# ateme-developers/SVT-AV1-1

Measured on AMD Instinct MI355X. Metric: 64x64 SAD-search blocks/sec, higher is better.
Workload: dtype u8; 1 GPU; configs[1]: 64x64 full-pel SAD hierarchical ME (centre check + HME L0/L1/L2 + 64x64-area full-pel search of 85 square PUs), 1080p 8-bit, one reference list

## Files before the change

### svt-av1-1_amd/csrc/me_fullpel.hip

```cpp
#include <hip/hip_runtime.h>
#include <stdint.h>

#include "me_kernels.h"
#include "me_wave_reduce.h"

namespace svthip {

namespace {
#include "me_fullpel_impl.h"
}

__global__ void __launch_bounds__(256, SVTHIP_FULLPEL_MIN_WAVES) fullpel85_kernel(
    const uint8_t* __restrict__ src_plane, uint32_t src_stride, const uint8_t* __restrict__ ref_plane,
    uint32_t ref_stride, const int32_t* __restrict__ desc, uint32_t n_sb, uint32_t* __restrict__ out_sad,
    uint32_t* __restrict__ out_mv)
{
    extern __shared__ __attribute__((aligned(16))) uint8_t smem[];
    const uint32_t sb = xcd_item(blockIdx.x, n_sb);
    if (sb >= n_sb) return;
    if ((desc[6 * sb + 4] & 15) == 0) fullpel85_sb<true>(src_plane, src_stride, ref_plane, ref_stride, desc + 6 * sb, sb, out_sad, out_mv, smem);
    else fullpel85_sb<false>(src_plane, src_stride, ref_plane, ref_stride, desc + 6 * sb, sb, out_sad, out_mv, smem);
}

}
```

### svt-av1-1_amd/csrc/me_fullpel_impl.h

```cpp
#pragma once


constexpr int kPitch = SVTHIP_FULLPEL_LDS_PITCH;

__device__ __forceinline__ uint64_t pack64(uint32_t lo, uint32_t hi) { return ((uint64_t)hi << 32) | lo; }

struct __attribute__((packed, aligned(1))) unaligned_u32 { uint32_t v; };
struct __attribute__((packed, aligned(1))) unaligned_u32x4 { uint32_t v[4]; };

__device__ __forceinline__ uint32_t min3u(uint32_t a, uint32_t b, uint32_t c)
{
    uint32_t r;
    asm("v_min3_u32 %0, %1, %2, %3" : "=v"(r) : "v"(a), "v"(b), "v"(c));
    return r;
}

__device__ __forceinline__ uint32_t track4(uint32_t best, uint64_t acc, const uint32_t* idx, uint32_t himask)
{
    const uint32_t lo = (uint32_t)acc, hi = (uint32_t)(acc >> 32);
    uint32_t k0 = (lo << 16) | idx[0];
    uint32_t k1 = (lo & himask) | idx[1];
    uint32_t k2 = (hi << 16) | idx[2];
    uint32_t k3 = (hi & himask) | idx[3];
    best = min3u(best, k0, k1);
    best = min3u(best, k2, k3);
    return best;
}

__device__ __forceinline__ uint32_t pk_min_u16(uint32_t a, uint32_t b)
{
    uint32_t r;
    asm("v_pk_min_u16 %0, %1, %2" : "=v"(r) : "v"(a), "v"(b));
    return r;
}

__device__ __forceinline__ uint32_t wave_min_u32(uint32_t v)
{
#pragma unroll
    for (int m = 1; m < 64; m <<= 1) {
        uint32_t o = __shfl_xor(v, m);
        v = o < v ? o : v;
    }
    return v;
}

__device__ __forceinline__ unsigned long long wave_min_u64(unsigned long long v)
{
#pragma unroll
    for (int m = 1; m < 64; m <<= 1) {
        unsigned long long o = __shfl_xor(v, m);
        v = o < v ? o : v;
    }
    return v;
}

__device__ __forceinline__ uint32_t mv_word(int x, int y)
{
    return ((uint32_t)(uint16_t)(y * 4) << 16) | (uint32_t)(uint16_t)(x * 4);
}


template <bool CLS>
__device__ __forceinline__ void fullpel85_sb(const uint8_t* __restrict__ src_plane, uint32_t src_stride,
                                             const uint8_t* __restrict__ ref_plane, uint32_t ref_stride, const int32_t* d, uint32_t sbi,
                                             uint32_t* __restrict__ out_sad, uint32_t* __restrict__ out_mv, uint8_t* smem)
{
    uint32_t* xch = reinterpret_cast<uint32_t*>(smem);
    unsigned long long* best64_lds = reinterpret_cast<unsigned long long*>(smem + 16384);
    uint8_t* win = smem + 16384 + 64;

    const int tid = threadIdx.x;
    const int lane = tid & 63;
    const int Q = __builtin_amdgcn_readfirstlane(tid >> 6);
    const int Qx = Q & 1, Qy = Q >> 1;

    const int src_off = __builtin_amdgcn_readfirstlane(d[0]);
    const int ref_off = __builtin_amdgcn_readfirstlane(d[1]);
    const int xo = __builtin_amdgcn_readfirstlane(d[2]), yo = __builtin_amdgcn_readfirstlane(d[3]);
    const int sw = __builtin_amdgcn_readfirstlane(d[4]), sh = __builtin_amdgcn_readfirstlane(d[5]);
    const int n_xg = (sw + 15) >> 4;
    const uint32_t inv_xg = (65536u + (uint32_t)n_xg - 1u) / (uint32_t)n_xg;

#ifdef SVTHIP_FP_STAGE_PRIO
    __builtin_amdgcn_s_setprio(3);
#endif
    {
        const uint8_t* base = ref_plane + ref_off;
        const int rows = sh + 63;
        const int ndw_valid = (sw + 63 + 3) >> 2;
        constexpr int q_row = kPitch >> 4;
        const int total = rows * q_row;
        for (int i = tid; i < total; i += 256) {
            const int r = i / q_row;
            const int c4 = i - r * q_row;
            const uint8_t* p = base + (size_t)r * ref_stride + 16 * c4;
            const int left = ndw_valid - 4 * c4;
            uint32_t t[4] = {0u, 0u, 0u, 0u};
            if (left >= 4) {
                const unaligned_u32x4 u = *reinterpret_cast<const unaligned_u32x4*>(p);
                t[0] = u.v[0]; t[1] = u.v[1]; t[2] = u.v[2]; t[3] = u.v[3];
            } else if (left > 0) {
#pragma unroll
                for (int k = 0; k < 3; k++)
                    if (k < left) t[k] = reinterpret_cast<const unaligned_u32*>(p + 4 * k)->v;
            }
            reinterpret_cast<uint4*>(win)[i] = make_uint4(t[0], t[1], t[2], t[3]);
        }
        if (tid == 0) *best64_lds = ~0ull;
    }
    __syncthreads();
#ifdef SVTHIP_FP_STAGE_PRIO
    __builtin_amdgcn_s_setprio(0);
#endif

    const uint32_t* src4 = reinterpret_cast<const uint32_t*>(src_plane + src_off + (size_t)(32 * Qy) * src_stride + 32 * Qx);
    const int sstride4 = src_stride >> 2;

    uint32_t rsv[4][2] = {{0, 0}, {0, 0}, {0, 0}, {0, 0}};
    if constexpr (CLS) {
        const int p = lane >> 2, zz = p >> 2, k = p & 3, px = 16 * (zz & 1) + 8 * (k & 1), py = 16 * (zz >> 1) + 8 * (k >> 1);
        const uint32_t* sp = src4 + (size_t)py * sstride4 + (px >> 2);
#pragma unroll
        for (int r = 0; r < 4; r++) {
            rsv[r][0] = sp[(size_t)(2 * r) * sstride4];
            rsv[r][1] = sp[(size_t)(2 * r) * sstride4 + 1];
        }
    }

    uint32_t best8[16], best16[4], best32 = 0xffffffffu;
#pragma unroll
    for (int i = 0; i < 16; i++) best8[i] = 0xffffffffu;
#pragma unroll
    for (int i = 0; i < 4; i++) best16[i] = 0xffffffffu;
    uint32_t best64_raw = 0xffffffffu, best64_idx = 0;

    const uint32_t himask = 0xffff0000u;
    const int n_items = n_xg * sh;
    const int n_iter = (n_items + 63) >> 6;

    for (int it = 0; it < n_iter; it++) {
        int pg = it * 64 + lane;
        const bool lane_valid = pg < n_items;
        if (!lane_valid) pg = 0;
        const int y = (int)(((uint32_t)pg * inv_xg) >> 16);
        const int xg = pg - y * n_xg;

        uint32_t idx[16];
        const uint32_t idx0 = (uint32_t)(y * 128 + 16 * xg);
        if ((sw & 15) == 0) {
#pragma unroll
            for (int i = 0; i < 16; i++) idx[i] = idx0 + (uint32_t)i;
        } else {
#pragma unroll
            for (int i = 0; i < 16; i++) idx[i] = (16 * xg + i < sw) ? idx0 + (uint32_t)i : 0xffffffffu;
        }

        uint32_t s16lo[4][4], s16hi[4][4];

        const uint8_t* wbase = win + (y + 32 * Qy) * kPitch + 16 * xg + 32 * Qx;

        uint4 An, Bn;
        uint32_t Sn[4];
        {
            An = *reinterpret_cast<const uint4*>(wbase);
            Bn = *reinterpret_cast<const uint4*>(wbase + 16);
#pragma unroll
            for (int h = 0; h < 4; h++) Sn[h] = src4[h];
        }
#pragma unroll
        for (int zz = 0; zz < 4; zz++) {
            uint64_t acc[4][4];

#pragma unroll
            for (int r8 = 0; r8 < 8; r8++) {
                const uint4 A = An, B = Bn;
                const uint32_t W[8] = {A.x, A.y, A.z, A.w, B.x, B.y, B.z, B.w};
                const uint32_t S[4] = {Sn[0], Sn[1], Sn[2], Sn[3]};
                asm volatile("" ::"v"(A.x), "v"(A.y), "v"(A.z), "v"(A.w), "v"(B.x), "v"(B.y), "v"(B.z), "v"(B.w), "s"(S[0]), "s"(S[1]), "s"(S[2]), "s"(S[3]));
                __builtin_amdgcn_sched_barrier(0);
                {
                    const int nstep = zz * 8 + r8 + 1;
                    if (nstep < 32) {
                        const int nzz = nstep >> 3, nr8 = nstep & 7, nC = nzz & 1, nR = nzz >> 1;
                        const uint8_t* p = wbase + (16 * nR + 2 * nr8) * kPitch + 16 * nC;
                        An = *reinterpret_cast<const uint4*>(p);
                        Bn = *reinterpret_cast<const uint4*>(p + 16);
                        const uint32_t* srow = src4 + (16 * nR + 2 * nr8) * sstride4 + 4 * nC;
#pragma unroll
                        for (int h = 0; h < 4; h++) Sn[h] = srow[h];
                    }
                    __builtin_amdgcn_sched_barrier(0);
                }
                const int krow = (r8 >> 2) * 2;
#pragma unroll
                for (int q = 0; q < 4; q++)
#pragma unroll
                    for (int h = 0; h < 4; h++) {
                        const int k = krow + (h >> 1);
                        const bool first = ((r8 & 3) == 0) && ((h & 1) == 0);
                        acc[k][q] = __builtin_amdgcn_qsad_pk_u16_u8(pack64(W[q + h], W[q + h + 1]), S[h],
                                                                    first ? 0ull : acc[k][q]);
                    }
            }

#pragma unroll
            for (int k = 0; k < 4; k++) {
                if constexpr (CLS) {
                    const uint32_t mlo = pk_min_u16(pk_min_u16((uint32_t)acc[k][0], (uint32_t)acc[k][1]), pk_min_u16((uint32_t)acc[k][2], (uint32_t)acc[k][3]));
                    const uint32_t mhi = pk_min_u16(pk_min_u16((uint32_t)(acc[k][0] >> 32), (uint32_t)(acc[k][1] >> 32)),
                                                    pk_min_u16((uint32_t)(acc[k][2] >> 32), (uint32_t)(acc[k][3] >> 32)));
                    best8[4 * zz + k] = track4(best8[4 * zz + k], pack64(mlo, mhi), &idx[0], himask);
                } else {
#pragma unroll
                    for (int q = 0; q < 4; q++) best8[4 * zz + k] = track4(best8[4 * zz + k], acc[k][q], &idx[4 * q], himask);
                }
            }

#pragma unroll
            for (int q = 0; q < 4; q++) {
                const uint32_t lo = (uint32_t)acc[0][q] + (uint32_t)acc[1][q] + (uint32_t)acc[2][q] + (uint32_t)acc[3][q];
                const uint32_t hi = (uint32_t)(acc[0][q] >> 32) + (uint32_t)(acc[1][q] >> 32) +
                                    (uint32_t)(acc[2][q] >> 32) + (uint32_t)(acc[3][q] >> 32);
                best16[zz] = track4(best16[zz], pack64(lo, hi), &idx[4 * q], himask);
                s16lo[zz][q] = lo;
                s16hi[zz][q] = hi;
            }
        }

        uint32_t s32acc[16];
#pragma unroll
        for (int q = 0; q < 4; q++) {
            const uint32_t a_lo = s16lo[0][q] + s16lo[1][q], b_lo = s16lo[2][q] + s16lo[3][q];
            const uint32_t a_hi = s16hi[0][q] + s16hi[1][q], b_hi = s16hi[2][q] + s16hi[3][q];
            s32acc[4 * q + 0] = (a_lo & 0xffffu) + (b_lo & 0xffffu);
            s32acc[4 * q + 1] = (a_lo >> 16) + (b_lo >> 16);
            s32acc[4 * q + 2] = (a_hi & 0xffffu) + (b_hi & 0xffffu);
            s32acc[4 * q + 3] = (a_hi >> 16) + (b_hi >> 16);
        }

#pragma unroll
        for (int i = 0; i < 16; i += 2) {
            uint32_t k0 = (s32acc[i] << 14) | idx[i];
            uint32_t k1 = (s32acc[i + 1] << 14) | idx[i + 1];
            best32 = min3u(best32, k0, k1);
        }

        __syncthreads();
        {
            uint4* dst = reinterpret_cast<uint4*>(xch + Q * 1024 + lane * 4);
#pragma unroll
            for (int q = 0; q < 4; q++) dst[q * 64] = make_uint4(s32acc[4 * q], s32acc[4 * q + 1], s32acc[4 * q + 2], s32acc[4 * q + 3]);
        }
        __syncthreads();
        {
            uint4 s = make_uint4(0, 0, 0, 0);
#pragma unroll
            for (int w = 0; w < 4; w++) {
                const uint4 v = *reinterpret_cast<const uint4*>(xch + w * 1024 + Q * 256 + lane * 4);
                s.x += v.x; s.y += v.y; s.z += v.z; s.w += v.w;
            }
            const uint32_t sv[4] = {s.x, s.y, s.z, s.w};
            const int xbase = 16 * xg + 4 * Q;
            const uint32_t ibase = (uint32_t)(y * 128 + xbase);
#pragma unroll
            for (int j = 0; j < 4; j++) {
                const bool better = (sv[j] < best64_raw) && lane_valid && (xbase + j < sw);
                best64_raw = better ? sv[j] : best64_raw;
                best64_idx = better ? (ibase + j) : best64_idx;
            }
        }
    }

    uint32_t* osad = out_sad + (size_t)85 * sbi;
    uint32_t* omv = out_mv + (size_t)85 * sbi;

    const uint32_t g8 = wave_min_scatter<16>(best8, lane);
    const uint32_t top[8] = {best16[0], best16[1], best16[2], best16[3], best32, 0xffffffffu, 0xffffffffu, 0xffffffffu};
    const uint32_t g16 = wave_min_scatter<8, 5>(top, lane);
    const unsigned long long k64 = wave_min_u64(((unsigned long long)best64_raw << 32) | best64_idx);

    if constexpr (CLS) {
        const int p = lane >> 2, q = lane & 3;
        const uint32_t key = (uint32_t)__shfl((int)g8, p);
        const uint32_t s = key >> 16, id = key & 0xffffu;
        const int y = (int)(id >> 7), xb = (int)(id & 0x70u);
        const int zz = p >> 2, k = p & 3, px = 16 * (zz & 1) + 8 * (k & 1), py = 16 * (zz >> 1) + 8 * (k >> 1);
        const uint8_t* wp = win + (y + 32 * Qy + py) * kPitch + xb + 4 * q + 32 * Qx + px;
        uint64_t a = 0;
#pragma unroll
        for (int r = 0; r < 4; r++) {
            const uint32_t* w = reinterpret_cast<const uint32_t*>(wp + 2 * r * kPitch);
            const uint32_t w0 = w[0], w1 = w[1], w2 = w[2];
            a = __builtin_amdgcn_qsad_pk_u16_u8(pack64(w0, w1), rsv[r][0], a);
            a = __builtin_amdgcn_qsad_pk_u16_u8(pack64(w1, w2), rsv[r][1], a);
        }
        const uint32_t lo = (uint32_t)a, hi = (uint32_t)(a >> 32);
        uint32_t first = (lo & 0xffffu) == s ? 0u : (lo >> 16) == s ? 1u : (hi & 0xffffu) == s ? 2u : (hi >> 16) == s ? 3u : 64u;
        first += 4u * (uint32_t)q;
        first = min(first, (uint32_t)__shfl_xor((int)first, 1));
        first = min(first, (uint32_t)__shfl_xor((int)first, 2));
        if (q == 0) {
            const int pu = 21 + 16 * Q + p;
            osad[pu] = 2u * s;
            omv[pu] = mv_word(xo + xb + (int)first, yo + y);
        }
    }
    if (lane < 21 && !(CLS && lane < 16)) {
        const uint32_t key = lane < 16 ? g8 : g16;
        const int pu = lane < 16 ? 21 + 16 * Q + lane : lane < 20 ? 5 + 4 * Q + (lane - 16) : 1 + Q;
        const uint32_t raw = lane == 20 ? key >> 14 : key >> 16, id = key & 0x3fffu;
        osad[pu] = 2u * raw;
        omv[pu] = mv_word(xo + (int)(id & 127u), yo + (int)(id >> 7));
    }
    if (lane == 0) atomicMin(best64_lds, k64);
    __syncthreads();
    if (tid == 0) {
        const unsigned long long k = *best64_lds;
        const uint32_t raw = (uint32_t)(k >> 32), id = (uint32_t)k;
        osad[0] = 2u * raw;
        omv[0] = mv_word(xo + (int)(id & 127u), yo + (int)(id >> 7));
    }
}
```

### svt-av1-1_amd/csrc/svthip_abi.hip

```cpp
#include <hip/hip_runtime.h>
#include <stdint.h>
#include <stdio.h>
#include <stdlib.h>
#include <string.h>

#include <mutex>
#include <new>

#include "../../include/svtav1_hip.h"
#include "me_kernels.h"

namespace {

thread_local char g_err[512] = "";

int32_t fail(int32_t code, const char* fmt, const char* a = "", int b = 0)
{
    snprintf(g_err, sizeof(g_err), fmt, a, b);
    return code;
}

#define HIP_TRY(expr)                                                                              \
    do {                                                                                           \
        hipError_t e_ = (expr);                                                                    \
        if (e_ != hipSuccess) return fail(SVTHIP_ERR_DEVICE, "%s failed at line %d", hipGetErrorString(e_), __LINE__); \
    } while (0)

}

struct svthip_ctx {
    int device;
    hipStream_t stream;
    void* scratch[18];
    size_t scratch_bytes[18];
    hipStream_t inter_stream;
    hipStream_t scratch_stream;
    hipEvent_t scratch_event;
    int32_t opt[SVTHIP_OPT_COUNT];
    uint32_t sb_table_w, sb_table_h;
};

namespace {

std::once_flag g_attr_once[16];
hipError_t g_attr_status[16];

void set_kernel_attrs(int device)
{
    const void* kernels[] = {reinterpret_cast<const void*>(svthip::fullpel85_kernel),  reinterpret_cast<const void*>(svthip::fullpel209_kernel),
                             reinterpret_cast<const void*>(svthip::bipred_pack_kernel), reinterpret_cast<const void*>(svthip::bipred_nsq_pack_kernel),
                             reinterpret_cast<const void*>(svthip::subpel_planes_kernel), svthip::convolve_compound_kernel_ptr(0),
                             svthip::convolve_compound_kernel_ptr(1),                     svthip::convolve_compound_kernel_ptr(2),
                             svthip::convolve_compound_kernel_ptr(3),                     svthip::convolve_compound_count_kernel_ptr(0),
                             svthip::convolve_compound_count_kernel_ptr(1),               svthip::convolve_compound_count_kernel_ptr(2),
                             svthip::convolve_compound_count_kernel_ptr(3)};
    hipError_t st = hipSuccess;
    for (const void* k : kernels) {
        hipFuncAttributes fa;
        hipError_t e = hipFuncGetAttributes(&fa, k);
        if (e == hipSuccess) e = hipFuncSetAttribute(k, hipFuncAttributeMaxDynamicSharedMemorySize, 160 * 1024 - (int)fa.sharedSizeBytes);
        if (e != hipSuccess) st = e;
    }
    g_attr_status[device] = st;
}

int32_t enter(svthip_ctx* c)
{
    if (!c) return fail(SVTHIP_ERR_BAD_PARAMETER, "null context%s", "");
    HIP_TRY(hipSetDevice(c->device));
    return SVTHIP_OK;
}
#define ENTER(ctx)                         \
    do {                                   \
        int32_t rc_ = enter(ctx);          \
        if (rc_) return rc_;               \
    } while (0)

int32_t scratch_on_stream(svthip_ctx* c, hipStream_t s)
{
    if (c->scratch_stream && c->scratch_stream != s) {
        HIP_TRY(hipEventRecord(c->scratch_event, c->scratch_stream));
        HIP_TRY(hipStreamWaitEvent(s, c->scratch_event, 0));
    }
    c->scratch_stream = s;
    return SVTHIP_OK;
}

int32_t ensure_scratch(svthip_ctx* c, int slot, size_t bytes)
{
    if (c->scratch_bytes[slot] >= bytes) return SVTHIP_OK;
    hipStream_t os = c->scratch_stream ? c->scratch_stream : c->stream;
    if (c->scratch[slot] && hipFreeAsync(c->scratch[slot], os) != hipSuccess) {
        (void)hipGetLastError();
        HIP_TRY(hipFree(c->scratch[slot]));
    }
    c->scratch[slot] = nullptr;
    c->scratch_bytes[slot] = 0;
    size_t want = bytes + bytes / 4 + 4096;
    if (hipMallocAsync(&c->scratch[slot], want, os) != hipSuccess) {
        (void)hipGetLastError();
        c->scratch[slot] = nullptr;
        return fail(SVTHIP_ERR_INSUFFICIENT_RESOURCES, "hipMallocAsync of %s scratch failed (slot %d)", "device", slot);
    }
    c->scratch_bytes[slot] = want;
    c->scratch_stream = os;
    if (slot == 9) {
        c->sb_table_w = c->sb_table_h = 0;
        HIP_TRY(hipMemsetAsync(c->scratch[9], 0, want, os));
    }
    return SVTHIP_OK;
}

size_t me_chain_bytes(size_t n, uint32_t n_pu)
{
    const size_t desc_b = sizeof(svthip_fullpel_desc) * n, arr_b = sizeof(uint32_t) * n_pu * n;
    const size_t state_b = ((sizeof(int16_t) * SVTHIP_HME_STATE_INT16 * n) + 15) & ~(size_t)15;
    return 2 * desc_b + 4 * arr_b + state_b + 64;
}
size_t me_pred_bytes(size_t n, uint32_t n_pu) { return 2 * (size_t)(n_pu == 209 ? 14 : 4) * 4096 * n; }

struct HostPoolLayout {
    uint32_t fs, qs, ss;
    size_t fb, qb, sb, per;
};
HostPoolLayout host_pool_layout(uint32_t w, uint32_t h)
{
    auto al = [](size_t v) { return (v + 15) & ~(size_t)15; };
    HostPoolLayout L;
    L.fs = w + 136; L.qs = (w >> 1) + 64; L.ss = (w >> 2) + 32;
    L.fb = al((size_t)L.fs * (h + 136)); L.qb = al((size_t)L.qs * ((h >> 1) + 64)); L.sb = al((size_t)L.ss * ((h >> 2) + 32));
    L.per = L.fb + L.qb + L.sb;
    return L;
}

int32_t ensure_sb_table(svthip_ctx* c, uint32_t w, uint32_t h, hipStream_t s)
{
    const uint32_t nx = (w + 63) / 64, ny = (h + 63) / 64, n_sb = nx * ny;
    int32_t rc;
    if ((rc = ensure_scratch(c, 9, sizeof(svthip_sb_origin) * n_sb))) return rc;
    if (c->sb_table_w == w && c->sb_table_h == h) return SVTHIP_OK;
    svthip_sb_origin* sbs = new (std::nothrow) svthip_sb_origin[n_sb];
    if (!sbs) return fail(SVTHIP_ERR_INSUFFICIENT_RESOURCES, "out of host memory%s", "");
    for (uint32_t y = 0; y < ny; y++)
        for (uint32_t x = 0; x < nx; x++) sbs[y * nx + x] = svthip_sb_origin{(uint16_t)(x * 64), (uint16_t)(y * 64)};
    hipError_t e = hipMemcpyAsync(c->scratch[9], sbs, sizeof(svthip_sb_origin) * n_sb, hipMemcpyHostToDevice, s);
    if (e == hipSuccess) e = hipStreamSynchronize(s);
    delete[] sbs;
    HIP_TRY(e);
    c->sb_table_w = w;
    c->sb_table_h = h;
    return SVTHIP_OK;
}

int32_t launch_fullpel(svthip_ctx* ctx, const uint8_t* d_src, uint32_t src_stride, const uint8_t* d_ref, uint32_t ref_stride,
                       const svthip_fullpel_desc* d_desc, uint32_t n_sb, uint32_t max_sw, uint32_t max_sh,
                       uint32_t* d_sad, uint32_t* d_mv, hipStream_t s)
{
    ENTER(ctx);
    if (n_sb == 0) return SVTHIP_OK;
    if (!d_src || !d_ref || !d_desc || !d_sad || !d_mv) return fail(SVTHIP_ERR_BAD_PARAMETER, "null pointer argument%s", "");
    if (max_sw < 1 || max_sw > 127 || max_sh < 1 || max_sh > 127)
        return fail(SVTHIP_ERR_BAD_PARAMETER, "search area must be 1..127 (%s%d)", "got ", (int)(max_sw > max_sh ? max_sw : max_sh));
    if ((src_stride & 3u) || (ref_stride & 3u) || (reinterpret_cast<uintptr_t>(d_src) & 3u))
        return fail(SVTHIP_ERR_BAD_PARAMETER, "plane strides and the source plane base must be multiples of 4%s", "");
    const size_t lds = svthip::fullpel_lds_bytes(max_sh);
    hipLaunchKernelGGL(svthip::fullpel85_kernel, dim3(svthip::xcd_grid(n_sb)), dim3(256), lds, s, d_src, src_stride, d_ref, ref_stride,
                       reinterpret_cast<const int32_t*>(d_desc), n_sb, d_sad, d_mv);
    HIP_TRY(hipGetLastError());
    return SVTHIP_OK;
}

}

extern "C" {

const char* svthip_last_error(void) { return g_err; }

int32_t svthip_create(int32_t device, svthip_ctx** out_ctx)
{
    if (!out_ctx) return fail(SVTHIP_ERR_BAD_PARAMETER, "out_ctx is null%s", "");
    *out_ctx = nullptr;
    int n = 0;
    if (hipGetDeviceCount(&n) != hipSuccess || n <= 0)
        return fail(SVTHIP_ERR_DEVICE, "no HIP device available%s (this library has no CPU fallback)", "");
    if (device < 0 || device >= n) return fail(SVTHIP_ERR_BAD_PARAMETER, "device index out of range%s (%d)", "", device);
    if (device >= 16) return fail(SVTHIP_ERR_BAD_PARAMETER, "device index above 15 is not supported%s (%d)", "", device);
    HIP_TRY(hipSetDevice(device));
    std::call_once(g_attr_once[device], set_kernel_attrs, device);
    if (g_attr_status[device] != hipSuccess)
        return fail(SVTHIP_ERR_DEVICE, "raising the kernels' dynamic LDS limit failed: %s", hipGetErrorString(g_attr_status[device]));
    svthip_ctx* c = new (std::nothrow) svthip_ctx();
    if (!c) return fail(SVTHIP_ERR_INSUFFICIENT_RESOURCES, "out of host memory%s", "");
    memset(c, 0, sizeof(*c));
    c->device = device;
    if (hipStreamCreateWithFlags(&c->stream, hipStreamNonBlocking) != hipSuccess) {
        delete c;
        return fail(SVTHIP_ERR_DEVICE, "hipStreamCreate failed%s", "");
    }
    if (hipEventCreateWithFlags(&c->scratch_event, hipEventDisableTiming) != hipSuccess) {
        (void)hipStreamDestroy(c->stream);
        delete c;
        return fail(SVTHIP_ERR_DEVICE, "hipEventCreate failed%s", "");
    }
    *out_ctx = c;
    return SVTHIP_OK;
}

void svthip_destroy(svthip_ctx* ctx)
{
    if (!ctx) return;
    (void)hipSetDevice(ctx->device);
    (void)hipStreamSynchronize(ctx->stream);
    for (int i = 0; i < 18; i++)
        if (ctx->scratch[i]) (void)hipFree(ctx->scratch[i]);
    (void)hipEventDestroy(ctx->scratch_event);
    (void)hipStreamDestroy(ctx->stream);
    delete ctx;
}

void* svthip_stream(svthip_ctx* ctx) { return ctx ? (void*)ctx->stream : nullptr; }

int32_t svthip_synchronize(svthip_ctx* ctx)
{
    ENTER(ctx);
    HIP_TRY(hipStreamSynchronize(ctx->stream));
    return SVTHIP_OK;
}

int32_t svthip_set_option(svthip_ctx* ctx, int32_t option, int32_t value)
{
    if (!ctx) return fail(SVTHIP_ERR_BAD_PARAMETER, "null context%s", "");
    if (option < 0 || option >= SVTHIP_OPT_COUNT) return fail(SVTHIP_ERR_BAD_PARAMETER, "unknown option%s %d", "", (int)option);
    ctx->opt[option] = value;
    return SVTHIP_OK;
}

int32_t svthip_reserve(svthip_ctx* ctx, uint32_t width, uint32_t height, uint32_t n_pu, uint32_t n_jobs, int32_t host_forms)
{
    ENTER(ctx);
    if ((width & 7) || (height & 7) || !width || !height || width > 16384 || height > 16384)
        return fail(SVTHIP_ERR_BAD_PARAMETER, "picture dimensions must be non-zero multiples of 8%s (width %d)", "", (int)width);
    if (n_pu != 85 && n_pu != 209) return fail(SVTHIP_ERR_BAD_PARAMETER, "n_pu must be 85 or 209%s (got %d)", "", (int)n_pu);
    if (n_jobs == 0) n_jobs = 1;
    const size_t n_sb = (size_t)((width + 63) / 64) * ((height + 63) / 64), n = n_sb * n_jobs;
    int32_t rc;
    if ((rc = ensure_scratch(ctx, 5, me_chain_bytes(n, n_pu)))) return rc;
    if ((rc = ensure_scratch(ctx, 6, sizeof(uint32_t) * 85 * n))) return rc;
    if ((rc = ensure_scratch(ctx, 7, me_pred_bytes(n, n_pu)))) return rc;
    if (host_forms) {
        const HostPoolLayout L = host_pool_layout(width, height);
        if ((rc = ensure_scratch(ctx, 8, L.per * 3 + 256))) return rc;
        if ((rc = ensure_scratch(ctx, 9, sizeof(svthip_sb_origin) * n_sb))) return rc;
        if ((rc = ensure_scratch(ctx, 10, sizeof(svthip_me_cu_result) * n_sb * n_pu))) return rc;
        if ((rc = ensure_scratch(ctx, 11, sizeof(svthip_me_cu_result_ref) * n_sb * n_pu))) return rc;
    }
    return SVTHIP_OK;
}

int32_t svthip_me_fullpel_search_dev(svthip_ctx* ctx, const uint8_t* d_src_plane, uint32_t src_stride,
                                     const uint8_t* d_ref_plane, uint32_t ref_stride, const svthip_fullpel_desc* d_desc,
                                     uint32_t n_sb, uint32_t max_search_area_width, uint32_t max_search_area_height,
                                     uint32_t* d_best_sad, uint32_t* d_best_mv, void* stream)
{
    ENTER(ctx);
    hipStream_t s = stream ? (hipStream_t)stream : ctx->stream;
    return launch_fullpel(ctx, d_src_plane, src_stride, d_ref_plane, ref_stride, d_desc, n_sb, max_search_area_width,
                          max_search_area_height, d_best_sad, d_best_mv, s);
}

static int32_t subpel_refine_common(svthip_ctx* ctx, const uint8_t* d_src_plane, uint32_t src_stride, const uint8_t* d_ref_plane,
                                     uint32_t ref_stride, const svthip_fullpel_desc* d_desc, uint32_t n_sb, uint32_t max_search_area_width,
                                     uint32_t max_search_area_height, int32_t disable_8x8_refinement, int n_pu, uint32_t* d_best_sad,
                                     uint32_t* d_best_mv, void* stream, uint32_t* d_pred = nullptr,
                                     int32_t method = SVTHIP_FRACTIONAL_SSD_SEARCH)
{
    ENTER(ctx);
    if (method != SVTHIP_FRACTIONAL_SUB_SAD_SEARCH && method != SVTHIP_FRACTIONAL_FULL_SAD_SEARCH && method != SVTHIP_FRACTIONAL_SSD_SEARCH)
        return fail(SVTHIP_ERR_BAD_PARAMETER, "fractional_search_method must be 0 (SUB_SAD), 1 (FULL_SAD) or 2 (SSD)%s, got %d", "", (int)method);
    if (n_sb == 0) return SVTHIP_OK;
    if (!d_src_plane || !d_ref_plane || !d_desc || !d_best_sad || !d_best_mv)
        return fail(SVTHIP_ERR_BAD_PARAMETER, "null pointer argument%s", "");
    if (max_search_area_width < 1 || max_search_area_width > 127 || max_search_area_height < 1 || max_search_area_height > 127)
        return fail(SVTHIP_ERR_BAD_PARAMETER, "search area must be 1..127%s", "");
    if ((src_stride & 3u) || (ref_stride & 3u) || (reinterpret_cast<uintptr_t>(d_src_plane) & 3u))
        return fail(SVTHIP_ERR_BAD_PARAMETER, "plane strides and the source plane base must be multiples of 4%s", "");
    hipStream_t s = stream ? (hipStream_t)stream : ctx->stream;
    const size_t lds_planes = svthip::subpel_planes_lds_bytes(max_search_area_width, max_search_area_height);
    if (lds_planes > 160 * 1024 - 512) return fail(SVTHIP_ERR_BAD_PARAMETER, "search area too large for the LDS planes%s", "");
    hipLaunchKernelGGL(svthip::subpel_planes_kernel, dim3(svthip::subpel_planes_grid(n_sb)), dim3(n_pu == 209 ? 448 : 512), lds_planes, s, d_src_plane, src_stride,
                       d_ref_plane, ref_stride, reinterpret_cast<const int32_t*>(d_desc), n_sb, (int)(disable_8x8_refinement != 0), n_pu,
                       d_best_sad, d_best_mv, d_pred, (int)method);
    HIP_TRY(hipGetLastError());
    return SVTHIP_OK;
}

int32_t svthip_me_subpel_refine_dev(svthip_ctx* ctx, const uint8_t* d_src_plane, uint32_t src_stride, const uint8_t* d_ref_plane,
                                    uint32_t ref_stride, const svthip_fullpel_desc* d_desc, uint32_t n_sb,
                                    uint32_t max_search_area_width, uint32_t max_search_area_height,
                                    int32_t disable_8x8_refinement, uint32_t* d_best_sad, uint32_t* d_best_mv, void* stream)
{
    return subpel_refine_common(ctx, d_src_plane, src_stride, d_ref_plane, ref_stride, d_desc, n_sb, max_search_area_width,
                                max_search_area_height, disable_8x8_refinement, 85, d_best_sad, d_best_mv, stream);
}

int32_t svthip_me_subpel_refine209_dev(svthip_ctx* ctx, const uint8_t* d_src_plane, uint32_t src_stride, const uint8_t* d_ref_plane,
                                       uint32_t ref_stride, const svthip_fullpel_desc* d_desc, uint32_t n_sb,
                                       uint32_t max_search_area_width, uint32_t max_search_area_height,
                                       int32_t disable_8x8_refinement, uint32_t* d_best_sad, uint32_t* d_best_mv, void* stream)
{
    return subpel_refine_common(ctx, d_src_plane, src_stride, d_ref_plane, ref_stride, d_desc, n_sb, max_search_area_width,
                                max_search_area_height, disable_8x8_refinement, 209, d_best_sad, d_best_mv, stream);
}

int32_t svthip_me_subpel_search_dev(svthip_ctx* ctx, const uint8_t* d_src_plane, uint32_t src_stride, const uint8_t* d_ref_plane,
                                    uint32_t ref_stride, const svthip_fullpel_desc* d_desc, uint32_t n_sb, uint32_t max_search_area_width,
                                    uint32_t max_search_area_height, int32_t disable_8x8_refinement, int32_t all_pu,
                                    int32_t fractional_search_method, uint32_t* d_best_sad, uint32_t* d_best_mv, void* stream)
{
    return subpel_refine_common(ctx, d_src_plane, src_stride, d_ref_plane, ref_stride, d_desc, n_sb, max_search_area_width,
                                max_search_area_height, disable_8x8_refinement, all_pu ? 209 : 85, d_best_sad, d_best_mv, stream, nullptr,
                                fractional_search_method);
}

static int32_t bipred_pack_common(svthip_ctx* ctx, const uint8_t* d_src_plane, uint32_t src_stride, const uint8_t* d_ref0_plane,
                                  uint32_t ref0_stride, const svthip_fullpel_desc* d_desc0, const uint8_t* d_ref1_plane,
                                  uint32_t ref1_stride, const svthip_fullpel_desc* d_desc1, uint32_t n_sb,
                                  uint32_t max_search_area_width, uint32_t max_search_area_height, const uint32_t* d_sad0,
                                  const uint32_t* d_mv0, const uint32_t* d_sad1, const uint32_t* d_mv1, uint32_t n_lists,
                                  int32_t bipred_8x8, int n_pu, svthip_me_cu_result* d_out, void* stream)
{
    ENTER(ctx);
    if (n_sb == 0) return SVTHIP_OK;
    if (n_lists < 1 || n_lists > 2) return fail(SVTHIP_ERR_BAD_PARAMETER, "n_lists must be 1 or 2%s", "");
    if (!d_sad0 || !d_mv0 || !d_out) return fail(SVTHIP_ERR_BAD_PARAMETER, "null pointer argument%s", "");
    size_t lds = 0, lds_nsq = 0;
    int win_bytes = 0;
    if (n_lists == 2) {
        if (!d_src_plane || !d_ref0_plane || !d_ref1_plane || !d_desc0 || !d_desc1 || !d_sad1 || !d_mv1)
            return fail(SVTHIP_ERR_BAD_PARAMETER, "null pointer argument%s", "");
        if (max_search_area_width < 1 || max_search_area_width > 127 || max_search_area_height < 1 || max_search_area_height > 127)
            return fail(SVTHIP_ERR_BAD_PARAMETER, "search area must be 1..127%s", "");
        if ((src_stride & 3u) || (ref0_stride & 3u) || (ref1_stride & 3u) || (reinterpret_cast<uintptr_t>(d_src_plane) & 3u))
            return fail(SVTHIP_ERR_BAD_PARAMETER, "plane strides and the source plane base must be multiples of 4%s", "");
        lds = svthip::bipred_lds_bytes(max_search_area_width, max_search_area_height);
        lds_nsq = svthip::bipred_nsq_lds_bytes(max_search_area_width, max_search_area_height);
        win_bytes = (int)svthip::subpel_window_bytes(max_search_area_width, max_search_area_height);
        if (lds > 160 * 1024 || (n_pu == 209 && lds_nsq > 160 * 1024))
            return fail(SVTHIP_ERR_BAD_PARAMETER, "search area too large for the LDS windows%s", "");
    }
    hipStream_t s = stream ? (hipStream_t)stream : ctx->stream;
    if (n_pu == 85) {
        hipLaunchKernelGGL(svthip::bipred_pack_kernel, dim3(n_sb), dim3(256), lds, s, d_src_plane, src_stride, d_ref0_plane, ref0_stride,
                           reinterpret_cast<const int32_t*>(d_desc0), d_ref1_plane, ref1_stride, reinterpret_cast<const int32_t*>(d_desc1),
                           d_sad0, d_mv0, d_sad1, d_mv1, (int)n_lists, (int)bipred_8x8, win_bytes, 85, (uint32_t*)nullptr, d_out);
        HIP_TRY(hipGetLastError());
        return SVTHIP_OK;
    }
    uint32_t* bisad_sq = nullptr;
    if (n_lists == 2) {
        int32_t rc;
        if ((rc = ensure_scratch(ctx, 6, sizeof(uint32_t) * 85 * (size_t)n_sb))) return rc;
        if ((rc = scratch_on_stream(ctx, s))) return rc;
        bisad_sq = static_cast<uint32_t*>(ctx->scratch[6]);
        hipLaunchKernelGGL(svthip::bipred_pack_kernel, dim3(n_sb), dim3(256), lds, s, d_src_plane, src_stride, d_ref0_plane, ref0_stride,
                           reinterpret_cast<const int32_t*>(d_desc0), d_ref1_plane, ref1_stride, reinterpret_cast<const int32_t*>(d_desc1),
                           d_sad0, d_mv0, d_sad1, d_mv1, 2, 1, win_bytes, 209, bisad_sq, (svthip_me_cu_result*)nullptr);
        HIP_TRY(hipGetLastError());
    }
    hipLaunchKernelGGL(svthip::bipred_nsq_pack_kernel, dim3(n_sb), dim3(320), lds_nsq, s, d_src_plane, src_stride, d_ref0_plane, ref0_stride,
                       reinterpret_cast<const int32_t*>(d_desc0), d_ref1_plane, ref1_stride, reinterpret_cast<const int32_t*>(d_desc1),
                       d_sad0, d_mv0, d_sad1, d_mv1, (int)n_lists, win_bytes, (const uint32_t*)bisad_sq, d_out);
    HIP_TRY(hipGetLastError());
    return SVTHIP_OK;
}

int32_t svthip_me_bipred_pack_dev(svthip_ctx* ctx, const uint8_t* d_src_plane, uint32_t src_stride, const uint8_t* d_ref0_plane,
                                  uint32_t ref0_stride, const svthip_fullpel_desc* d_desc0, const uint8_t* d_ref1_plane,
                                  uint32_t ref1_stride, const svthip_fullpel_desc* d_desc1, uint32_t n_sb,
                                  uint32_t max_search_area_width, uint32_t max_search_area_height, const uint32_t* d_sad0,
                                  const uint32_t* d_mv0, const uint32_t* d_sad1, const uint32_t* d_mv1, uint32_t n_lists,
                                  int32_t bipred_8x8, svthip_me_cu_result* d_out, void* stream)
{
    return bipred_pack_common(ctx, d_src_plane, src_stride, d_ref0_plane, ref0_stride, d_desc0, d_ref1_plane, ref1_stride, d_desc1, n_sb,
                              max_search_area_width, max_search_area_height, d_sad0, d_mv0, d_sad1, d_mv1, n_lists, bipred_8x8, 85, d_out,
                              stream);
}

int32_t svthip_me_bipred_pack209_dev(svthip_ctx* ctx, const uint8_t* d_src_plane, uint32_t src_stride, const uint8_t* d_ref0_plane,
                                     uint32_t ref0_stride, const svthip_fullpel_desc* d_desc0, const uint8_t* d_ref1_plane,
                                     uint32_t ref1_stride, const svthip_fullpel_desc* d_desc1, uint32_t n_sb,
                                     uint32_t max_search_area_width, uint32_t max_search_area_height, const uint32_t* d_sad0,
                                     const uint32_t* d_mv0, const uint32_t* d_sad1, const uint32_t* d_mv1, uint32_t n_lists,
                                     svthip_me_cu_result* d_out, void* stream)
{
    return bipred_pack_common(ctx, d_src_plane, src_stride, d_ref0_plane, ref0_stride, d_desc0, d_ref1_plane, ref1_stride, d_desc1, n_sb,
                              max_search_area_width, max_search_area_height, d_sad0, d_mv0, d_sad1, d_mv1, n_lists, 1, 209, d_out, stream);
}

int32_t svthip_quantize_b_batch_dev(svthip_ctx* ctx, const int32_t* d_coeff, const svthip_quant_desc* d_desc, uint32_t n_tu,
                                    const int16_t* d_qparams, const int16_t* d_iscan, int32_t* d_qcoeff, int32_t* d_dqcoeff,
                                    uint16_t* d_eob, void* stream)
{
    ENTER(ctx);
    if (n_tu == 0) return SVTHIP_OK;
    if (!d_coeff || !d_desc || !d_qparams || !d_iscan || !d_qcoeff || !d_dqcoeff || !d_eob)
        return fail(SVTHIP_ERR_BAD_PARAMETER, "null pointer argument%s", "");
    if ((reinterpret_cast<uintptr_t>(d_coeff) | reinterpret_cast<uintptr_t>(d_qcoeff) | reinterpret_cast<uintptr_t>(d_dqcoeff)) & 15u)
        return fail(SVTHIP_ERR_BAD_PARAMETER, "coefficient pools must be 16-byte aligned%s", "");
    if (reinterpret_cast<uintptr_t>(d_iscan) & 7u) return fail(SVTHIP_ERR_BAD_PARAMETER, "iscan pool must be 8-byte aligned%s", "");
    hipStream_t s = stream ? (hipStream_t)stream : ctx->stream;
    const uint32_t waves = n_tu < 8192u ? n_tu : 8192u;
    hipLaunchKernelGGL(svthip::quantize_b_batch_kernel, dim3((waves + 3) / 4), dim3(256), 0, s, d_coeff, d_desc, n_tu, d_qparams,
                       d_iscan, d_qcoeff, d_dqcoeff, d_eob);
    HIP_TRY(hipGetLastError());
    return SVTHIP_OK;
}

int32_t svthip_me_fullpel_search209_dev(svthip_ctx* ctx, const uint8_t* d_src_plane, uint32_t src_stride, const uint8_t* d_ref_plane,
                                        uint32_t ref_stride, const svthip_fullpel_desc* d_desc, uint32_t n_sb,
                                        uint32_t max_search_area_width, uint32_t max_search_area_height, uint32_t* d_best_sad,
                                        uint32_t* d_best_mv, void* stream)
{
    ENTER(ctx);
    if (n_sb == 0) return SVTHIP_OK;
    if (!d_src_plane || !d_ref_plane || !d_desc || !d_best_sad || !d_best_mv) return fail(SVTHIP_ERR_BAD_PARAMETER, "null pointer argument%s", "");
    if (max_search_area_width < 1 || max_search_area_width > 127 || max_search_area_height < 1 || max_search_area_height > 127)
        return fail(SVTHIP_ERR_BAD_PARAMETER, "search area must be 1..127 (%s%d)", "got ",
                    (int)(max_search_area_width > max_search_area_height ? max_search_area_width : max_search_area_height));
    if ((src_stride & 3u) || (ref_stride & 3u) || (reinterpret_cast<uintptr_t>(d_src_plane) & 3u))
        return fail(SVTHIP_ERR_BAD_PARAMETER, "plane strides and the source plane base must be multiples of 4%s", "");
    const size_t lds = svthip::fullpel209_lds_bytes(max_search_area_height);
    hipStream_t s = stream ? (hipStream_t)stream : ctx->stream;
    hipLaunchKernelGGL(svthip::fullpel209_kernel, dim3(svthip::xcd_grid(n_sb)), dim3(256), lds, s, d_src_plane, src_stride, d_ref_plane, ref_stride,
                       reinterpret_cast<const int32_t*>(d_desc), n_sb, d_best_sad, d_best_mv);
    HIP_TRY(hipGetLastError());
    return SVTHIP_OK;
}

int32_t svthip_fwd_txfm2d_batch_dev(svthip_ctx* ctx, const int16_t* d_residual, const svthip_txfm_desc* d_desc, uint32_t n_tu,
                                    uint32_t tx_width, uint32_t tx_height, uint32_t bit_depth, int32_t* d_coeff, void* stream)
{
    ENTER(ctx);
    if (!svthip::fwd_txfm2d_size_valid((int)tx_width, (int)tx_height))
        return fail(SVTHIP_ERR_BAD_PARAMETER, "unsupported transform size%s (width %d)", "", (int)tx_width);
    if (bit_depth != 8 && bit_depth != 10) return fail(SVTHIP_ERR_BAD_PARAMETER, "bit_depth must be 8 or 10%s (got %d)", "", (int)bit_depth);
    if (n_tu == 0) return SVTHIP_OK;
    if (!d_residual || !d_desc || !d_coeff) return fail(SVTHIP_ERR_BAD_PARAMETER, "null pointer argument%s", "");
    if (reinterpret_cast<uintptr_t>(d_coeff) & 15u) return fail(SVTHIP_ERR_BAD_PARAMETER, "coefficient pool must be 16-byte aligned%s", "");
    hipStream_t s = stream ? (hipStream_t)stream : ctx->stream;
    HIP_TRY(svthip::launch_fwd_txfm2d(d_residual, d_desc, n_tu, (int)tx_width, (int)tx_height, d_coeff, s));
    return SVTHIP_OK;
}

int32_t svthip_inv_txfm2d_add_batch_dev(svthip_ctx* ctx, const int32_t* d_coeff, const svthip_itxfm_desc* d_desc, uint32_t n_tu,
                                        uint32_t tx_width, uint32_t tx_height, uint32_t bit_depth, uint32_t recon_16bit,
                                        void* d_recon, void* stream)
{
    ENTER(ctx);
    if (!svthip::fwd_txfm2d_size_valid((int)tx_width, (int)tx_height))
        return fail(SVTHIP_ERR_BAD_PARAMETER, "unsupported transform size%s (width %d)", "", (int)tx_width);
    if (bit_depth != 8 && bit_depth != 10) return fail(SVTHIP_ERR_BAD_PARAMETER, "bit_depth must be 8 or 10%s (got %d)", "", (int)bit_depth);
    if (bit_depth == 10 && !recon_16bit) return fail(SVTHIP_ERR_BAD_PARAMETER, "10-bit reconstruction needs a 16-bit plane%s", "");
    if (n_tu == 0) return SVTHIP_OK;
    if (!d_coeff || !d_desc || !d_recon) return fail(SVTHIP_ERR_BAD_PARAMETER, "null pointer argument%s", "");
    if (reinterpret_cast<uintptr_t>(d_coeff) & 15u) return fail(SVTHIP_ERR_BAD_PARAMETER, "coefficient pool must be 16-byte aligned%s", "");
    if (recon_16bit && (reinterpret_cast<uintptr_t>(d_recon) & 1u)) return fail(SVTHIP_ERR_BAD_PARAMETER, "16-bit plane must be 2-byte aligned%s", "");
    hipStream_t s = stream ? (hipStream_t)stream : ctx->stream;
    HIP_TRY(svthip::launch_inv_txfm2d_add(d_coeff, d_desc, n_tu, (int)tx_width, (int)tx_height, (int)bit_depth, d_recon,
                                          recon_16bit ? 1 : 0, s));
    return SVTHIP_OK;
// ... 749 lines not shown
```

Measured before the change: 9.493 million blocks/s.

## Add two-image LDS layout kernel for 64-wide full-pel search windows

Adds a specialised full-pel kernel for search areas up to 64x64. It stages a second copy of the reference window, shifted by 4 bytes, so the odd-offset 64-bit operands for qsad come straight from aligned 128-bit LDS reads instead of being repacked from neighbouring registers. It also maps lanes to fixed rows and x-groups through a lookup table, which removes the per-item divide and bounds masking. The cost is twice the LDS footprint, a longer staging phase and more live registers, which may lower occupancy.

```diff
diff --git a/svt-av1-1_amd/csrc/me_fullpel.hip b/svt-av1-1_amd/csrc/me_fullpel.hip
--- a/svt-av1-1_amd/csrc/me_fullpel.hip
+++ b/svt-av1-1_amd/csrc/me_fullpel.hip
@@ -1,6 +1,7 @@
 #include <hip/hip_runtime.h>
 #include <stdint.h>
 
+#include "me_fullpel_img2.h"
 #include "me_kernels.h"
 #include "me_wave_reduce.h"
 
@@ -22,4 +23,18 @@
     else fullpel85_sb<false>(src_plane, src_stride, ref_plane, ref_stride, desc + 6 * sb, sb, out_sad, out_mv, smem);
 }
 
+__global__ void __launch_bounds__(256, SVTHIP_FULLPEL_MIN_WAVES) fullpel85_img2_kernel(
+    const uint8_t* __restrict__ src_plane, uint32_t src_stride, const uint8_t* __restrict__ ref_plane,
+    uint32_t ref_stride, const int32_t* __restrict__ desc, uint32_t n_sb, uint32_t* __restrict__ out_sad,
+    uint32_t* __restrict__ out_mv)
+{
+    extern __shared__ __attribute__((aligned(16))) uint8_t smem[];
+    const uint32_t sb = xcd_item(blockIdx.x, n_sb);
+    if (sb >= n_sb) return;
+    const int sw = desc[6 * sb + 4];
+    if (sw == 64) fullpel85_sb<true, true>(src_plane, src_stride, ref_plane, ref_stride, desc + 6 * sb, sb, out_sad, out_mv, smem);
+    else if ((sw & 15) == 0) fullpel85_sb<true>(src_plane, src_stride, ref_plane, ref_stride, desc + 6 * sb, sb, out_sad, out_mv, smem);
+    else fullpel85_sb<false>(src_plane, src_stride, ref_plane, ref_stride, desc + 6 * sb, sb, out_sad, out_mv, smem);
 }
+
+}
diff --git a/svt-av1-1_amd/csrc/me_fullpel_img2.h b/svt-av1-1_amd/csrc/me_fullpel_img2.h
--- /dev/null
+++ b/svt-av1-1_amd/csrc/me_fullpel_img2.h
@@ -0,0 +1,23 @@
+#pragma once
+#include "me_kernels.h"
+
+#define SVTHIP_FULLPEL_IMG2_PITCH 144
+#define SVTHIP_FULLPEL_IMG2_ROWS 127
+#define SVTHIP_FULLPEL_IMG2_MAX_AREA 64
+
+namespace svthip {
+
+__global__ void fullpel85_img2_kernel(const uint8_t* __restrict__ src_plane, uint32_t src_stride, const uint8_t* __restrict__ ref_plane,
+                                      uint32_t ref_stride, const int32_t* __restrict__ desc, uint32_t n_sb, uint32_t* __restrict__ out_sad,
+                                      uint32_t* __restrict__ out_mv);
+
+inline bool fullpel_img2_fits(uint32_t max_sw, uint32_t max_sh)
+{
+    return max_sw <= SVTHIP_FULLPEL_IMG2_MAX_AREA && max_sh <= SVTHIP_FULLPEL_IMG2_MAX_AREA;
+}
+inline size_t fullpel_img2_lds_bytes()
+{
+    return SVTHIP_FULLPEL_LDS_FIXED + 2 * (size_t)SVTHIP_FULLPEL_IMG2_ROWS * SVTHIP_FULLPEL_IMG2_PITCH;
+}
+
+}
diff --git a/svt-av1-1_amd/csrc/me_fullpel_impl.h b/svt-av1-1_amd/csrc/me_fullpel_impl.h
--- a/svt-av1-1_amd/csrc/me_fullpel_impl.h
+++ b/svt-av1-1_amd/csrc/me_fullpel_impl.h
@@ -2,8 +2,18 @@
 
 
 constexpr int kPitch = SVTHIP_FULLPEL_LDS_PITCH;
+constexpr int kPitch2 = SVTHIP_FULLPEL_IMG2_PITCH;
+constexpr int kImage1 = SVTHIP_FULLPEL_IMG2_ROWS * SVTHIP_FULLPEL_IMG2_PITCH;
+constexpr unsigned long long kRowLut = 0xFEAB6732DC894510ull;
 
 __device__ __forceinline__ uint64_t pack64(uint32_t lo, uint32_t hi) { return ((uint64_t)hi << 32) | lo; }
+
+typedef uint32_t u32x4_t __attribute__((ext_vector_type(4)));
+__device__ __forceinline__ uint4 lds_read_b128(const uint8_t* p)
+{
+    const u32x4_t v = *(const volatile __attribute__((address_space(3))) u32x4_t*)p;
+    return make_uint4(v.x, v.y, v.z, v.w);
+}
 
 struct __attribute__((packed, aligned(1))) unaligned_u32 { uint32_t v; };
 struct __attribute__((packed, aligned(1))) unaligned_u32x4 { uint32_t v[4]; };
@@ -60,7 +70,7 @@
 }
 
 
-template <bool CLS>
+template <bool CLS, bool IMG2 = false>
 __device__ __forceinline__ void fullpel85_sb(const uint8_t* __restrict__ src_plane, uint32_t src_stride,
                                              const uint8_t* __restrict__ ref_plane, uint32_t ref_stride, const int32_t* d, uint32_t sbi,
                                              uint32_t* __restrict__ out_sad, uint32_t* __restrict__ out_mv, uint8_t* smem)
@@ -68,6 +78,8 @@
     uint32_t* xch = reinterpret_cast<uint32_t*>(smem);
     unsigned long long* best64_lds = reinterpret_cast<unsigned long long*>(smem + 16384);
     uint8_t* win = smem + 16384 + 64;
+    static_assert(!IMG2 || CLS, "the two-image form is a form of the class loop");
+    constexpr int P = IMG2 ? kPitch2 : kPitch;
 
     const int tid = threadIdx.x;
     const int lane = tid & 63;
@@ -88,23 +100,27 @@
         const uint8_t* base = ref_plane + ref_off;
         const int rows = sh + 63;
         const int ndw_valid = (sw + 63 + 3) >> 2;
-        constexpr int q_row = kPitch >> 4;
+        constexpr int q_row = P >> 4;
         const int total = rows * q_row;
+        auto slot = [](const uint8_t* p, int left) {
+            uint32_t t[4] = {0u, 0u, 0u, 0u};
+            if (left >= 4) {
+                const unaligned_u32x4 u = *reinterpret_cast<const unaligned_u32x4*>(p);
+                t[0] = u.v[0]; t[1] = u.v[1]; t[2] = u.v[2]; t[3] = u.v[3];
+            } else if (left > 0) {
+#pragma unroll
+                for (int k = 0; k < 3; k++)
+                    if (k < left) t[k] = reinterpret_cast<const unaligned_u32*>(p + 4 * k)->v;
+            }
+            return make_uint4(t[0], t[1], t[2], t[3]);
+        };
         for (int i = tid; i < total; i += 256) {
             const int r = i / q_row;
             const int c4 = i - r * q_row;
             const uint8_t* p = base + (size_t)r * ref_stride + 16 * c4;
             const int left = ndw_valid - 4 * c4;
-            uint32_t t[4] = {0u, 0u, 0u, 0u};
-            if (left >= 4) {
-                const unaligned_u32x4 u = *reinterpret_cast<const unaligned_u32x4*>(p);
-                t[0] = u.v[0]; t[1] = u.v[1]; t[2] = u.v[2]; t[3] = u.v[3];
-            } else if (left > 0) {
-#pragma unroll
-                for (int k = 0; k < 3; k++)
-                    if (k < left) t[k] = reinterpret_cast<const unaligned_u32*>(p + 4 * k)->v;
-            }
-            reinterpret_cast<uint4*>(win)[i] = make_uint4(t[0], t[1], t[2], t[3]);
+            reinterpret_cast<uint4*>(win)[i] = slot(p, left);
+            if constexpr (IMG2) reinterpret_cast<uint4*>(win + kImage1)[i] = slot(p + 4, left - 1);
         }
         if (tid == 0) *best64_lds = ~0ull;
     }
@@ -136,18 +152,28 @@
 
     const uint32_t himask = 0xffff0000u;
     const int n_items = n_xg * sh;
-    const int n_iter = (n_items + 63) >> 6;
+    const int n_iter = IMG2 ? (sh + 15) >> 4 : (n_items + 63) >> 6;
+    const int lane_row = (int)((kRowLut >> (4 * (lane >> 2))) & 15u);
 
     for (int it = 0; it < n_iter; it++) {
-        int pg = it * 64 + lane;
-        const bool lane_valid = pg < n_items;
-        if (!lane_valid) pg = 0;
-        const int y = (int)(((uint32_t)pg * inv_xg) >> 16);
-        const int xg = pg - y * n_xg;
+        int y, xg;
+        bool lane_valid;
+        if constexpr (IMG2) {
+            y = 16 * it + lane_row;
+            xg = lane & 3;
+            lane_valid = y < sh;
+            if (!lane_valid) y = 0;
+        } else {
+            int pg = it * 64 + lane;
+            lane_valid = pg < n_items;
+            if (!lane_valid) pg = 0;
+            y = (int)(((uint32_t)pg * inv_xg) >> 16);
+            xg = pg - y * n_xg;
+        }
 
         uint32_t idx[16];
         const uint32_t idx0 = (uint32_t)(y * 128 + 16 * xg);
-        if ((sw & 15) == 0) {
+        if (IMG2 || (sw & 15) == 0) {
 #pragma unroll
             for (int i = 0; i < 16; i++) idx[i] = idx0 + (uint32_t)i;
         } else {
@@ -157,13 +183,20 @@
 
         uint32_t s16lo[4][4], s16hi[4][4];
 
-        const uint8_t* wbase = win + (y + 32 * Qy) * kPitch + 16 * xg + 32 * Qx;
-
-        uint4 An, Bn;
+        const uint8_t* wbase = win + (y + 32 * Qy) * P + 16 * xg + 32 * Qx;
+
+        uint4 An, Bn, Cn = make_uint4(0, 0, 0, 0), Dn = make_uint4(0, 0, 0, 0);
         uint32_t Sn[4];
         {
-            An = *reinterpret_cast<const uint4*>(wbase);
-            Bn = *reinterpret_cast<const uint4*>(wbase + 16);
+            if constexpr (IMG2) {
+                An = lds_read_b128(wbase);
+                Bn = lds_read_b128(wbase + 16);
+                Cn = lds_read_b128(wbase + kImage1);
+                Dn = lds_read_b128(wbase + kImage1 + 16);
+            } else {
+                An = *reinterpret_cast<const uint4*>(wbase);
+                Bn = *reinterpret_cast<const uint4*>(wbase + 16);
+            }
 #pragma unroll
             for (int h = 0; h < 4; h++) Sn[h] = src4[h];
         }
@@ -173,18 +206,29 @@
 
 #pragma unroll
             for (int r8 = 0; r8 < 8; r8++) {
-                const uint4 A = An, B = Bn;
+                const uint4 A = An, B = Bn, Cw = Cn, Dw = Dn;
                 const uint32_t W[8] = {A.x, A.y, A.z, A.w, B.x, B.y, B.z, B.w};
                 const uint32_t S[4] = {Sn[0], Sn[1], Sn[2], Sn[3]};
+                const uint64_t WP[7] = {pack64(W[0], W[1]), IMG2 ? pack64(Cw.x, Cw.y) : pack64(W[1], W[2]), pack64(W[2], W[3]),
+                                        IMG2 ? pack64(Cw.z, Cw.w) : pack64(W[3], W[4]), pack64(W[4], W[5]),
+                                        IMG2 ? pack64(Dw.x, Dw.y) : pack64(W[5], W[6]), pack64(W[6], W[7])};
                 asm volatile("" ::"v"(A.x), "v"(A.y), "v"(A.z), "v"(A.w), "v"(B.x), "v"(B.y), "v"(B.z), "v"(B.w), "s"(S[0]), "s"(S[1]), "s"(S[2]), "s"(S[3]));
+                if constexpr (IMG2) asm volatile("" ::"v"(Cw.x), "v"(Cw.y), "v"(Cw.z), "v"(Cw.w), "v"(Dw.x), "v"(Dw.y), "v"(Dw.z), "v"(Dw.w));
                 __builtin_amdgcn_sched_barrier(0);
                 {
                     const int nstep = zz * 8 + r8 + 1;
                     if (nstep < 32) {
                         const int nzz = nstep >> 3, nr8 = nstep & 7, nC = nzz & 1, nR = nzz >> 1;
-                        const uint8_t* p = wbase + (16 * nR + 2 * nr8) * kPitch + 16 * nC;
-                        An = *reinterpret_cast<const uint4*>(p);
-                        Bn = *reinterpret_cast<const uint4*>(p + 16);
+                        const uint8_t* p = wbase + (16 * nR + 2 * nr8) * P + 16 * nC;
+                        if constexpr (IMG2) {
+                            An = lds_read_b128(p);
+                            Bn = lds_read_b128(p + 16);
+                            Cn = lds_read_b128(p + kImage1);
+                            Dn = lds_read_b128(p + kImage1 + 16);
+                        } else {
+                            An = *reinterpret_cast<const uint4*>(p);
+                            Bn = *reinterpret_cast<const uint4*>(p + 16);
+                        }
                         const uint32_t* srow = src4 + (16 * nR + 2 * nr8) * sstride4 + 4 * nC;
 #pragma unroll
                         for (int h = 0; h < 4; h++) Sn[h] = srow[h];
@@ -198,8 +242,7 @@
                     for (int h = 0; h < 4; h++) {
                         const int k = krow + (h >> 1);
                         const bool first = ((r8 & 3) == 0) && ((h & 1) == 0);
-                        acc[k][q] = __builtin_amdgcn_qsad_pk_u16_u8(pack64(W[q + h], W[q + h + 1]), S[h],
-                                                                    first ? 0ull : acc[k][q]);
+                        acc[k][q] = __builtin_amdgcn_qsad_pk_u16_u8(WP[q + h], S[h], first ? 0ull : acc[k][q]);
                     }
             }
 
@@ -285,11 +328,11 @@
         const uint32_t s = key >> 16, id = key & 0xffffu;
         const int y = (int)(id >> 7), xb = (int)(id & 0x70u);
         const int zz = p >> 2, k = p & 3, px = 16 * (zz & 1) + 8 * (k & 1), py = 16 * (zz >> 1) + 8 * (k >> 1);
-        const uint8_t* wp = win + (y + 32 * Qy + py) * kPitch + xb + 4 * q + 32 * Qx + px;
+        const uint8_t* wp = win + (y + 32 * Qy + py) * P + xb + 4 * q + 32 * Qx + px;
         uint64_t a = 0;
 #pragma unroll
         for (int r = 0; r < 4; r++) {
-            const uint32_t* w = reinterpret_cast<const uint32_t*>(wp + 2 * r * kPitch);
+            const uint32_t* w = reinterpret_cast<const uint32_t*>(wp + 2 * r * P);
             const uint32_t w0 = w[0], w1 = w[1], w2 = w[2];
             a = __builtin_amdgcn_qsad_pk_u16_u8(pack64(w0, w1), rsv[r][0], a);
             a = __builtin_amdgcn_qsad_pk_u16_u8(pack64(w1, w2), rsv[r][1], a);
diff --git a/svt-av1-1_amd/csrc/svthip_abi.hip b/svt-av1-1_amd/csrc/svthip_abi.hip
--- a/svt-av1-1_amd/csrc/svthip_abi.hip
+++ b/svt-av1-1_amd/csrc/svthip_abi.hip
@@ -8,6 +8,7 @@
 #include <new>
 
 #include "../../include/svtav1_hip.h"
+#include "me_fullpel_img2.h"
 #include "me_kernels.h"
 
 namespace {
@@ -163,9 +164,14 @@
         return fail(SVTHIP_ERR_BAD_PARAMETER, "search area must be 1..127 (%s%d)", "got ", (int)(max_sw > max_sh ? max_sw : max_sh));
     if ((src_stride & 3u) || (ref_stride & 3u) || (reinterpret_cast<uintptr_t>(d_src) & 3u))
         return fail(SVTHIP_ERR_BAD_PARAMETER, "plane strides and the source plane base must be multiples of 4%s", "");
-    const size_t lds = svthip::fullpel_lds_bytes(max_sh);
-    hipLaunchKernelGGL(svthip::fullpel85_kernel, dim3(svthip::xcd_grid(n_sb)), dim3(256), lds, s, d_src, src_stride, d_ref, ref_stride,
-                       reinterpret_cast<const int32_t*>(d_desc), n_sb, d_sad, d_mv);
+    if (svthip::fullpel_img2_fits(max_sw, max_sh)) {
+        hipLaunchKernelGGL(svthip::fullpel85_img2_kernel, dim3(svthip::xcd_grid(n_sb)), dim3(256), svthip::fullpel_img2_lds_bytes(), s, d_src,
+                           src_stride, d_ref, ref_stride, reinterpret_cast<const int32_t*>(d_desc), n_sb, d_sad, d_mv);
+    } else {
+        const size_t lds = svthip::fullpel_lds_bytes(max_sh);
+        hipLaunchKernelGGL(svthip::fullpel85_kernel, dim3(svthip::xcd_grid(n_sb)), dim3(256), lds, s, d_src, src_stride, d_ref, ref_stride,
+                           reinterpret_cast<const int32_t*>(d_desc), n_sb, d_sad, d_mv);
+    }
     HIP_TRY(hipGetLastError());
     return SVTHIP_OK;
 }
```

Result: faster. 9.749 million blocks/s (median of 6 runs) (+2.7%).
